# iucario/WorkoutDetector

Hardware: AMD Instinct MI355X
Metric: clips/sec (8x3x224x224 TSM-R50) (higher is better)
Workload: dtype f32

## Files before the change

### workoutdetector_amd/csrc/tsm_conv_rules.h

```cpp
#pragma once
#include <stdint.h>
#include <string.h>

#if defined(__HIPCC__)
#define TSM_HOST_DEVICE __host__ __device__
#else
#define TSM_HOST_DEVICE
#endif

namespace tsm {

struct ConvParams {
  const float *x;
  const float *w;
  const float *bias;
  const float *res;
  float *y;
  int N, Hi, Wi, C, logC4;
  int Ho, Wo, Cout;
  int stride, pad;
  int Kp;
  int M;
  int relu;
  int T;
  int fold;
  int ntm, ntn;
  int tile;
  int prec;
  const float *x2;
  int C2, Hi2, Wi2, stride2;
  int K1;
  int kseg_len;
  int ksplit;
  int tail_from;
  float *ypart;
  int reverse;
  int pos_major;
};

enum ConvPrec { kPrecF32 = 0, kPrecBf16x3 = 1, kPrecBf16 = 2 };
constexpr int kPrecBlockShift = 4;
constexpr int kPrecPosMajor = 8;

enum ConvTile {
  kTileAuto = 0, kTile128x128 = 1, kTile128x64 = 2, kTile64x64 = 3, kTile32x32 = 4,
  kTile128x128w8 = 5,
  kTile256x256 = 6,
  kTileWs = 7,
  kTile256x256p = 8,
  kTile64x128 = 9,
  kNumTiles = 10
};

struct Fused23Params {
  const float *x;
  const float *w2;
  const float *bias2;
  const float *w3f;
  const float *bias3;
  const float *res;
// ... 292 lines not shown
    case kTile64x128:
      return p.prec == kPrecF32 && p.pad == 0 && p.kseg_len == 0 && p.Cout % 128 == 0 &&
             !(p.T > 0 && (p.res || p.x2 || p.stride != 1));
    case kTileWs: {
      int tr, tc;
      return conv3x3_ws_valid(p, &tr, &tc) || conv3x3_ws128s2_valid(p, &tr, &tc) || conv3x3_ws128_valid(p, &tr, &tc, nullptr) ||
             conv1x1_ws_valid(p) || conv1x1_wsn_valid(p, n_cu);
    }
    default: return false;
  }
}

enum ConvFamily { kFamInvalid = 0, kFamIgemm, kFamIgemmSeg, kFamBf16_256, kFamBf16_256p, kFamWs3x3, kFamWs128, kFamWs128s2, kFamWs1x1, kFamWsn };

struct ConvRoute {
  int family = kFamInvalid, ks = 0;
  int bm = 0, bn = 0, wgm = 0, wgn = 0;
  bool shift = false, res = false, dual = false, block_shift = false;
  bool pos_major = false;
  int ntm = 0, ntn = 0;
  long tiles = 0;
  unsigned grid = 0;
  int tr = 0, tc = 0, swz = 0;
};

inline bool conv_args_refused(const ConvParams &p, int ks) {
  const int kc = p.prec == kPrecBf16 ? 64 : kBK;
  if (p.Cout % 64 != 0 || p.Kp % kc != 0 || p.M <= 0) return true;
  if (p.logC4 < 0 || p.logC4 > 28 || (1 << p.logC4) * 4 != p.C) return true;
  if (ks != 7 && p.C % kc != 0) return true;
  if (p.T > 0 && ((ks != 1 && ks != 3) || (ks == 3 && p.kseg_len > 0) || p.N % p.T != 0 || p.fold % 4 != 0 ||
                  (p.res && 2 * (int64_t)p.fold > p.Cout) || (p.x2 && 2 * (int64_t)p.fold > p.C2)))
    return true;
  if (p.x2 && (ks != 1 || p.res || p.K1 % kc != 0 || p.C2 % kc != 0 || (int64_t)p.K1 + p.C2 != p.Kp || p.K1 != p.C))
    return true;
  if (p.x2 && (128.0 / ((double)p.Ho * p.Wo) + 4.0) * (double)p.Hi2 * p.Wi2 * p.C2 * 4.0 > 2.0e9) return true;
  if (p.T > 0 && p.res && (128.0 + 2.0 * p.Ho * p.Wo) * p.Cout * 4.0 > 2.0e9) return true;
  if (p.prec != kPrecF32 && p.prec != kPrecBf16x3 && p.prec != kPrecBf16) return true;
  if (p.kseg_len < 0 || (p.kseg_len > 0 && (p.prec != kPrecF32 || p.res || ks == 7))) return true;
  if ((p.ksplit && p.kseg_len <= 0) || p.ksplit < 0 || p.ksplit > 2) return true;
  if (p.prec != kPrecF32 && p.T > 0 && p.fold % 8 != 0) return true;
  if (ks == 7 && (p.C != 4 || (p.prec != kPrecF32 && (p.stride != 2 || p.pad != 3)))) return true;
  if ((128.0 / ((double)p.Ho * p.Wo) + 4.0) * (double)p.Hi * p.Wi * p.C * 4.0 > 2.0e9) return true;
  return (ks != 1 && ks != 3 && ks != 7) || (ks == 7 && p.res);
}

// ... 8 lines not shown
  for (int ky = 0; ky < 3; ++ky)
    for (int kx = 0; kx < 3; ++kx)
      if ((unsigned)(iy0 + ky) < (unsigned)Hi && (unsigned)(ix0 + kx) < (unsigned)Wi) mask |= 1u << (ky * 3 + kx);
  return mask;
}
TSM_HOST_DEVICE inline int next_live_kstep(int kt, unsigned mask, int steps_per_tap, int nk) {
  if (kt < 0 || kt >= nk) return nk;
  const int log_spt = __builtin_ctz((unsigned)steps_per_tap);
  const int tap = kt >> log_spt;
  const unsigned rest = tap < 9 ? (mask & 0x1ffu) >> tap : 0u;
  if (rest & 1u) return kt;
  if (rest == 0u) return nk;
  const int next = (tap + __builtin_ctz(rest)) << log_spt;
  return next < nk ? next : nk;
}
inline bool pos_major_valid(const ConvParams &p, int ks) {
  return p.prec == kPrecF32 && ks == 3 && p.pad == 1 && (p.stride == 1 || p.stride == 2) && p.kseg_len > 0 && p.T == 0 &&
         !p.res && !p.x2 && (p.tile == kTile64x64 || p.tile == kTileAuto) && (p.ksplit == 0 || p.ksplit == 2) &&
         p.N > 0 && p.N % 64 == 0 && p.Ho > 0 && p.Wo > 0 && (int64_t)p.N * p.Ho * p.Wo == p.M &&
         p.C >= kBK && (p.C & (p.C - 1)) == 0 && p.Kp == (int64_t)9 * p.C &&
         (double)p.N * p.Hi * p.Wi * p.C * 4.0 < 2.0e9 && (double)p.M * p.Cout * 4.0 < 2.0e9;
}

inline ConvRoute conv_route(const ConvParams &p, int ks, int n_cu) {
  ConvRoute r, refused;
  if (conv_args_refused(p, ks) || (p.tile != kTileAuto && !conv_tile_valid(p, p.tile, n_cu))) return refused;
  r.ks = ks; r.res = p.res != nullptr; r.dual = p.x2 != nullptr;
  r.shift = !r.res && p.T > 0 && !(ks == 1 && r.dual);
  if (p.tile == kTileAuto) conv_tile_shape(p, &r.bm, &r.bn);
  else conv_tile_dims(p.tile, &r.bm, &r.bn);
  if (p.tile == kTile256x256 || p.tile == kTile256x256p) {
    const bool persistent = p.tile == kTile256x256p;
    if (!(persistent ? conv_bf16_256p_valid(p, ks) : conv_bf16_256_valid(p, ks))) return refused;
    r.family = persistent ? kFamBf16_256p : kFamBf16_256;
    r.wgm = 2; r.wgn = 4;
    r.shift = ks == 1 && p.T > 0;
    r.ntm = (int)(((long)p.M + 255) / 256); r.ntn = p.Cout / 256;
    r.tiles = (long)r.ntm * r.ntn;
    const int slots = n_cu & ~7;
    r.grid = (unsigned)(!persistent || r.tiles < slots || slots < 8 ? r.tiles : slots);
    return r.tiles > 0x7fffffffL ? refused : r;
  }
  if (p.tile == kTileWs) {
    if (ks == 3) {
      r.family = conv3x3_ws128s2_valid(p, &r.tr, &r.tc) ? kFamWs128s2 : conv3x3_ws128_valid(p, &r.tr, &r.tc, &r.swz) ? kFamWs128 :
                 conv3x3_ws_valid(p, &r.tr, &r.tc) ? kFamWs3x3 : kFamInvalid;
// ... 7 lines not shown
      r.tiles = ((long)p.M + px - 1) / px;
    }
    r.grid = persistent_grid(r.tiles, n_cu);
    if (r.family == kFamWsn && p.x2 && p.Kp == 384) {
      const int pairs = n_cu >> 4 << 3;
      r.grid = 2u * (unsigned)(r.tiles < pairs ? (r.tiles + 7) / 8 * 8 : pairs);
    }
    return r;
  }
  if (p.tile == kTile64x128 && ks != 1) return refused;
  if (p.kseg_len > 0 && r.bm != 32) r.bm = r.bn = 64;
  if (r.bm == 32 && p.prec != kPrecF32) return refused;
  r.wgm = r.bm == 32 ? 1 : r.bm == 128 && r.bn == 128 && p.tile == kTile128x128w8 ? 4 : 2;
  r.wgn = r.bm == 32 ? 1 : 2;
  r.ntm = (int)(((long)p.M + r.bm - 1) / r.bm); r.ntn = p.Cout / r.bn;
  r.tiles = (long)r.ntm * r.ntn;
  long grid = r.tiles;
  if (p.kseg_len > 0) {
    if (r.res || ks == 7 || (r.shift && ks == 3)) return refused;
    if (p.ksplit == 2 && (p.tail_from <= 0 || p.tail_from >= r.tiles || p.tail_from % r.ntn != 0)) return refused;
    r.family = kFamIgemmSeg;
    r.pos_major = p.pos_major != 0 && r.bm == 64 && pos_major_valid(p, ks);
    grid = p.ksplit == 2 ? p.tail_from + (r.tiles - p.tail_from) * conv_num_segments(p) : r.tiles * (p.ksplit ? conv_num_segments(p) : 1);
  } else {
    r.family = kFamIgemm;
  }
  r.block_shift = p.T > 0 && (r.dual || r.res);
  r.grid = (unsigned)grid;
  return grid > 0x7fffffffL ? refused : r;
}

inline bool conv23_ws_valid(int n, int h, int w, int *tr_out = nullptr, int *tc_out = nullptr) {
  int tr, tc;
  return n > 0 && h > 0 && w > 0 && (double)h * w * 512.0 < 2.0e9 && (double)n * h * w < 2.0e9 &&
         ws_tile_geometry(h, w, tr_out ? tr_out : &tr, tc_out ? tc_out : &tc);
}
inline bool bneck_ws_valid(int cin, int n, int h, int w, int T, int fold) {
  return (cin == 256 || cin == 64) && n > 0 && h > 0 && w >= 1 && w <= 64 && (double)h * w * 512.0 * 3.0 < 2.0e9 &&
         (T == 0 || (T > 0 && n % T == 0 && fold == cin / 8));
}
inline bool front_s2_valid(int n, int h, int w, int T, int fold) {
  return n > 0 && h >= 2 && (h & 1) == 0 && w >= 2 && w <= 64 && (double)h * w * 512.0 * 3.0 < 2.0e9 &&
         (T == 0 || (T > 0 && n % T == 0 && fold == 32));
}
inline int conv31_rows(const Conv31Params &p) {
  if (p.K3 == 128 && p.C == 512 && p.N1 == 128) return 256;
// ... 13 lines not shown
```

### workoutdetector_amd/csrc/tsm_device.h

```cpp
#pragma once
#include "tsm_kernels.h"

#include <cstdio>
#include <cstdlib>
#include <cstring>
#include <map>
#include <mutex>
#include <utility>

namespace tsm {

typedef float f32x16 __attribute__((ext_vector_type(16)));
typedef float f32x4 __attribute__((ext_vector_type(4)));
typedef float f32x2 __attribute__((ext_vector_type(2)));
typedef unsigned u32x4 __attribute__((ext_vector_type(4)));

constexpr int kLds = 36;

constexpr unsigned kInvalid = 0x80000000u;

__device__ __forceinline__ long xcd_chunked(long v, long n) {
  const long q8 = n >> 3, r8 = n & 7, x = v & 7;
  return (x < r8 ? x * (q8 + 1) : r8 * (q8 + 1) + (x - r8) * q8) + (v >> 3);
}
// ... 84 lines not shown
}
#define TSM_STAMP_DECL(on, n) \
  [[maybe_unused]] unsigned long long stamp_acc[(on) ? (n) : 1] = {}, stamp_last = (on) ? __builtin_amdgcn_s_memtime() : 0
#define TSM_STAMP(on, i)                                          \
  do {                                                            \
    if (on) {                                                     \
      const unsigned long long _t = __builtin_amdgcn_s_memtime(); \
      stamp_acc[(on) ? (i) : 0] += _t - stamp_last;               \
      stamp_last = _t;                                            \
    }                                                             \
  } while (0)

#define TSM_KLAUNCH(kern, ...)                          \
  do {                                                  \
    ::tsm::note_launch(#kern, __PRETTY_FUNCTION__);     \
    hipLaunchKernelGGL(kern, __VA_ARGS__);              \
  } while (0)
#define TSM_KLAUNCH_WALK(rev, kern, ...)                             \
  do {                                                               \
    ::tsm::note_launch(#kern, __PRETTY_FUNCTION__, (rev) ? 1 : 0);   \
    hipLaunchKernelGGL(kern, __VA_ARGS__);                           \
  } while (0)

inline unsigned grid_for(int64_t total, int cap) {
  const int64_t blocks = (total + 255) / 256;
  return (unsigned)(blocks < cap ? (blocks > 0 ? blocks : 1) : cap);
}

struct DeviceInfo {
  int n_cu = 256;
  hipError_t status = hipSuccess;
};
const DeviceInfo &device_info();
hipError_t lds_opt_in(const void *kernel, size_t bytes);
struct OptIn {
  hipError_t first = hipSuccess;
  void operator()(const void *fn, size_t bytes) {
    const hipError_t st = lds_opt_in(fn, bytes);
    if (st != hipSuccess && first == hipSuccess) first = st;
  }
};
hipError_t opt_in_bf16_256();
hipError_t opt_in_ws();
hipError_t opt_in_bneck();
hipError_t opt_in_conv31();
hipError_t opt_in_front();
// ... 7 lines not shown
```

### workoutdetector_amd/csrc/tsm_engine.hip

```cpp
#include <hip/hip_runtime.h>

#include <sys/stat.h>

#include <algorithm>
#include <cerrno>
#include <cmath>
#include <cstdio>
#include <cstdlib>
#include <cstring>
#include <map>
#include <string>
#include <vector>

#include "../../include/tsm_hip.h"
#include "tsm_host_util.h"
#include "tsm_kernels.h"

#ifndef TSM_BUILD_ID
#define TSM_BUILD_ID __DATE__ "/" __TIME__
#endif

namespace {

using namespace tsm_host;
// ... 152 lines not shown
  float *buf[5] = {nullptr, nullptr, nullptr, nullptr, nullptr};
  float *d_pooled = nullptr, *d_logits = nullptr;
  float *d_partial = nullptr;
  size_t partial_elems = 0;
  size_t buf_elems = 0;
  int h1 = 0, w1 = 0, hp = 0, wp = 0;
  hipEvent_t ev0 = nullptr, ev1 = nullptr;
  bool have_time = false;
  std::vector<void *> allocs;
  bool poison = false;
  std::vector<GuardBuf> guards;
  std::map<int, std::vector<int>> tile_cache;
  bool autotune = true;
  bool stem_pool = true;
  bool stem_direct = true;
  bool stem_planar = true;
  std::string tune_path, tune_sig;
  int force_tile = 0, force_code = -1;
  int fuse23 = -1;
  int fuse_block = -1;
  int fuse31 = -1;
  int fuse_front = -1;
  bool pos_major = true;
  bool tile_64x128 = true;
  int walk = -1;
  int n_cu = 256;
  int timing_left = 0;
  bool timing_only3x3 = false;
  std::vector<std::vector<hipEvent_t>> timing;
  std::vector<hipEvent_t> event_pool;
  std::vector<hipEvent_t> *cur_timing = nullptr;
};

namespace {

int fail(tsm_engine *e, int code, const std::string &msg) {
  if (e) e->err = msg; else g_create_error = msg;
  return code;
}

#define TSM_HIP(e, call)                                                                        \
  do {                                                                                          \
    hipError_t _st = (call);                                                                    \
    if (_st != hipSuccess)                                                                      \
      return fail((e), TSM_ERR_HIP, std::string(#call) + ": " + hipGetErrorString(_st));        \
  } while (0)
// ... 320 lines not shown
  fclose(f);
  return ok;
}

void tune_cache_store(tsm_engine *e, int key, const std::vector<int> &codes) {
  if (e->tune_path.empty()) return;
  std::string line = e->tune_sig + "|" + std::to_string(key) + "|";
  for (size_t i = 0; i < codes.size(); ++i) line += (i ? "," : "") + std::to_string(codes[i]);
  line += "\n";
  if (line.size() >= 4096) return;
  FILE *f = fopen(e->tune_path.c_str(), "a");
  if (!f) return;
  fwrite(line.data(), 1, line.size(), f);
  fclose(f);
}

bool tail_split_from(const tsm::ConvParams &p, int n_cu, size_t partial_elems, int *tail_from) {
  if (p.kseg_len <= 0) return false;
  const long from = tsm_host::tail_split_point(p.M, p.Cout, tsm::conv_num_segments(p), n_cu, partial_elems);
  *tail_from = (int)from;
  return from > 0;
}

hipError_t launch_conv_code(tsm::ConvParams p, int ks, int code, float *partial, size_t partial_elems, int n_cu, hipStream_t s) {
  p.tile = code & kCodeTileMask;
  const bool pos_major = (code & kCodePosMajor) && !(code & kCodeSplitK) && (code & kCodeTileMask) == tsm::kTile64x64 &&
                         tsm::pos_major_valid(p, ks);
  p.pos_major = pos_major ? 1 : 0;
  if ((code & kCodeSplitK) && p.kseg_len > 0 &&
      (size_t)tsm::conv_num_segments(p) * (size_t)p.M * (size_t)p.Cout <= partial_elems) {
    float *y = p.y;
    p.ksplit = 1;
    p.y = partial;
    hipError_t st = tsm::launch_conv(p, ks, s);
    if (st == hipSuccess)
      st = tsm::launch_splitk_reduce(partial, tsm::conv_num_segments(p), p.M, p.Cout, p.bias, nullptr, y, p.relu, s);
    return st;
  }
  if ((code & kCodeTailK) && (code & kCodeTileMask) == tsm::kTile64x64 && p.kseg_len > 0) {
    int tail_from = 0;
    if (tail_split_from(p, n_cu, partial_elems, &tail_from)) {
      float *y = p.y;
      const int mt0 = tail_from / (p.Cout / 64) * 64;
      p.ksplit = 2;
      p.tail_from = tail_from;
      p.ypart = partial;
      hipError_t st = tsm::launch_conv(p, ks, s);
      if (st == hipSuccess && pos_major)
        st = tsm::launch_splitk_reduce_pos(partial, tsm::conv_num_segments(p), mt0, p.M - mt0, p.N, p.Ho * p.Wo, p.Cout, p.bias, y,
                                           p.relu, s);
      else if (st == hipSuccess)
// ... 199 lines not shown
  }
  hipError_t launch_code(tsm::ConvParams p, int ks, int code);
  hipError_t launch_pair(const tsm::ConvParams &a, int ks_a, int code_a, const tsm::ConvParams &b, int ks_b, int code_b) {
    const hipError_t st = launch_code(a, ks_a, code_a);
    return st != hipSuccess ? st : launch_code(b, ks_b, code_b);
  }
  template <class A, class B>
  int fused_wins(A &&many, B &&one, bool *wins) {
    float many_ms = 0.f, one_ms = 0.f;
    int rc = time_best_of(e, s, many, &many_ms);
    if (!rc) rc = time_best_of(e, s, one, &one_ms);
    *wins = one_ms < many_ms;
    return rc;
  }
  int conv(int idx, tsm::ConvParams p, int ks, bool is3x3);
  int run_basic(size_t k, int nn, float *x, float *y, int hh, int ww);
  int run_block(size_t k, const BlockPlan &plan, int nn, float *x, float *y, int hh, int ww);
  int run_nonlocal(size_t k, int nn, float *x, float *z, int hh, int ww);
  int run_mse(size_t k, int nn, int hh, int ww);
  int tune_block(size_t k, int nn, float *x, float *y, int hh, int ww);
};

hipError_t Forward::launch_code(tsm::ConvParams p, int ks, int code) {
  return launch_conv_code(p, ks, code, e->d_partial, e->partial_elems, e->n_cu, s);
}

int Forward::conv(int idx, tsm::ConvParams p, int ks, bool is3x3) {
  p.reverse = next_dir();
  if (!tuning) {
    int code = tiles ? (*tiles)[idx] : 0;
    if (e->force_tile) code = e->force_tile;
    if (e->force_code >= 0) code = e->force_code;
    TSM_LAUNCH_K(e, s, is3x3, launch_code(p, ks, checked_code(p, code, e->n_cu)));
    return TSM_OK;
  }
  std::vector<int> cands;
  if (p.kseg_len > 0) {
    const size_t need = (size_t)tsm::conv_num_segments(p) * p.M * p.Cout;
    const long tiles64 = (long)((p.M + 63) / 64) * (p.Cout / 64);
    for (int t : {(int)tsm::kTile64x64, (int)tsm::kTile32x32}) {
      cands.push_back(t);
      if (need <= e->partial_elems && tiles64 < 4L * e->n_cu) cands.push_back(t | kCodeSplitK);
    }
    int tail_from = 0;
    const bool tail = tail_split_from(p, e->n_cu, e->partial_elems, &tail_from);
    if (tail) cands.push_back((int)tsm::kTile64x64 | kCodeTailK);
    tsm::ConvParams q = p;
// ... 905 lines not shown
    if (rows >= (int64_t)1 << 31)
      return fail(nullptr, TSM_ERR_CAPACITY, "max_clips * num_segments * (H/2) * (W/2) must stay below 2^31");
  }
  if (const char *why = shift_div_refusal(cfg->shift_div, tsm::kPrecF32)) return fail(nullptr, TSM_ERR_UNSUPPORTED, why);
  if (prec_of_dtype(cfg->dtype) < 0)
    return fail(nullptr, TSM_ERR_UNSUPPORTED, "dtype must be TSM_DTYPE_F32, TSM_DTYPE_BF16X3 or TSM_DTYPE_BF16");
  if (const char *why = shift_div_refusal(cfg->shift_div, prec_of_dtype(cfg->dtype))) return fail(nullptr, TSM_ERR_UNSUPPORTED, why);
  int ndev = 0;
  hipError_t st = hipGetDeviceCount(&ndev);
  if (st != hipSuccess || ndev <= 0)
    return fail(nullptr, TSM_ERR_HIP, std::string("no HIP device: ") + hipGetErrorString(st));
  if (cfg->device_id < 0 || cfg->device_id >= ndev) return fail(nullptr, TSM_ERR_INVALID_ARG, "bad device_id");
  tsm_engine *e = new tsm_engine();
  e->cfg = *cfg;
  e->prec = prec_of_dtype(cfg->dtype);
  const auto on = [](const char *s) { return atoi(s) != 0; };
  env_read("TSM_AUTOTUNE", &e->autotune, on);
  env_read("TSM_STEM_DIRECT", &e->stem_direct, on);
  env_read("TSM_STEM_POOL", &e->stem_pool, on);
  env_read("TSM_STEM_PLANAR", &e->stem_planar, on);
  env_read("TSM_CONV_TILE", &e->force_tile, tsm::conv_tile_from_name);
  env_read("TSM_CONV_CODE", &e->force_code, atoi);
  env_read("TSM_POS_MAJOR", &e->pos_major, on);
  env_read("TSM_TILE_64X128", &e->tile_64x128, on);
  env_read("TSM_FUSE_CONV23", &e->fuse23, on);
  env_read("TSM_FUSE_BLOCK", &e->fuse_block, on);
  env_read("TSM_FUSE_C3C1", &e->fuse31, on);
  env_read("TSM_FUSE_FRONT", &e->fuse_front, on);
  env_read("TSM_WALK", &e->walk, on);
  env_read("TSM_POISON", &e->poison, on);
  const char *tc = getenv("TSM_TUNE_CACHE");
  if (!tc) e->tune_path = default_tune_cache_path();
  else if (*tc && strcmp(tc, "0") != 0 && strcmp(tc, "off") != 0) e->tune_path = tc;
  build_topology(e);
  st = hipSetDevice(cfg->device_id);
  if (st == hipSuccess) st = hipStreamCreateWithFlags(&e->stream, hipStreamNonBlocking);
  if (st == hipSuccess) st = hipDeviceGetAttribute(&e->n_cu, hipDeviceAttributeMultiprocessorCount, cfg->device_id);
  if (st == hipSuccess) st = hipEventCreate(&e->ev0);
  if (st == hipSuccess) st = hipEventCreate(&e->ev1);
  if (st != hipSuccess) {
    g_create_error = std::string("engine init: ") + hipGetErrorString(st);
    delete e;
    return TSM_ERR_HIP;
  }
  if (!e->tune_path.empty()) {
    hipDeviceProp_t prop;
// ... 494 lines not shown
    xin = d_x4;
  } else if (x3 && (rc = staged(a->x, "d_xs", (size_t)pl.x_elems, in_px * a->cin, &xin))) {
    return rc;
  }
  if (x3) {
    if ((rc = scratch.alloc(&d_ys, "d_ys", out_elems, out_frame, act_bytes))) return rc;
    yout = d_ys;
    if (rin && (rc = staged(rin, "d_rs", out_elems, out_frame, &rin))) return rc;
    if (pl.dual && (rc = staged(x2in, "d_x2s", (size_t)pl.x2_elems, (size_t)a->hi2 * a->wi2 * a->cin2, &x2in))) return rc;
  }
  tsm::ConvParams p = make_params(c, xin, rin, yout, n, hi, wi, a->relu != 0, pl.T, 1, prec);
  p.fold = pl.fold;
  p.reverse = a->reverse != 0;
  if (pl.dual) set_second_source(&p, c2.kp, x2in, a->cin2, a->hi2, a->wi2, a->stride2);
  int dev = 0, n_cu = 256;
  TSM_HIP(nullptr, hipGetDevice(&dev));
  TSM_HIP(nullptr, hipDeviceGetAttribute(&n_cu, hipDeviceAttributeMultiprocessorCount, dev));
  const int code = checked_code(p, a->code > 0 ? a->code & ~kCodeOpSegmented : a->code, n_cu);
  size_t part_elems = 0;
  if ((code & (kCodeSplitK | kCodeTailK)) && p.kseg_len > 0) {
    part_elems = (size_t)tsm::conv_num_segments(p) * p.M * p.Cout;
    if ((rc = scratch.alloc(&d_part, "d_part", part_elems, out_frame))) return rc;
  }
  const char *sd_env = getenv("TSM_STEM_DIRECT");
  hipError_t st;
  if (pl.stem && x3 && cout == 64 && !(sd_env && atoi(sd_env) == 0))
    st = tsm::launch_stem_direct(xin, c.d_w, c.d_b, yout, n, hi, wi, c.kp, a->relu != 0, prec, s);
  else
    st = launch_conv_code(p, a->k, code, d_part, part_elems, n_cu, s);
  if (st == hipSuccess && x3) st = tsm::launch_to_f32(d_ys, a->y, (int64_t)out_elems / 8, prec, s);
  const hipError_t st2 = hipStreamSynchronize(s);
  if (st != hipSuccess) return op_status("launch_conv", st);
  if (st2 != hipSuccess) return fail(nullptr, TSM_ERR_HIP, std::string("conv sync: ") + hipGetErrorString(st2));
  for (int i = 0; i < scratch.n; ++i) {
    std::string msg;
    TSM_HIP(nullptr, guard_verify(scratch.g[i], &msg));
    if (!msg.empty()) return fail(nullptr, TSM_ERR_GUARD, "tsm_conv_op: " + msg);
  }
  return TSM_OK;
}

int tsm_conv_bn_act(const float *x, const float *w, const float *gamma, const float *beta, const float *mean,
                    const float *var, const float *residual, float *y, int32_t n, int32_t hi, int32_t wi,
                    int32_t cin, int32_t cout, int32_t k, int32_t stride, int32_t relu, int32_t shift_segments,
                    int32_t fold_div, int32_t dtype, void *stream) {
  tsm_conv_args a{};
  a.struct_size = sizeof(tsm_conv_args);
  a.x = x; a.w = w; a.gamma = gamma; a.beta = beta; a.mean = mean; a.var = var; a.residual = residual; a.y = y;
  a.n = n; a.hi = hi; a.wi = wi; a.cin = cin; a.cout = cout; a.k = k; a.stride = stride; a.relu = relu;
  a.shift_segments = shift_segments; a.fold_div = fold_div; a.dtype = dtype;
  a.code = tsm::conv_tile_from_name(getenv("TSM_CONV_TILE"));
  return tsm_conv_op(&a, stream);
// ... 229 lines not shown
```

### workoutdetector_amd/csrc/tsm_igemm.hip

```cpp
#include "tsm_device.h"

namespace tsm {

template <int BM, int BN, int WGM, int WGN, int KS, bool SHIFT, bool RES, int PREC, bool DUAL = false, bool SEG = false>
__global__ void __launch_bounds__(64 * WGM * WGN, (SEG && BM == 64) ? ((PREC & kPrecBlockShift) ? 4 : 5) : (BM == 64 && BN == 128) ? 4 : 1)
conv_igemm(const ConvParams p) {
  constexpr bool BSHIFT = (PREC & kPrecBlockShift) != 0;
  constexpr bool POSM = (PREC & kPrecPosMajor) != 0;
  constexpr int PMODE = PREC & ~(kPrecBlockShift | kPrecPosMajor);
  static_assert(!POSM || (SEG && KS == 3 && BM == 64 && BN == 64 && !SHIFT && !RES && !DUAL && !BSHIFT && PMODE == kPrecF32),
                "position-major rows: the segmented fp32 3x3 on 64x64 tiles only (pos_major_valid)");
  static_assert(!BSHIFT || (!SHIFT && !RES), "block placement: a shifted identity (DUAL = false) or a shifted second source");
  constexpr bool RESID = RES || (BSHIFT && !DUAL);
  static_assert(!SEG || (PMODE == kPrecF32 && !RES && WGM * WGN <= 4 && BM == BN && BM <= 64),
                "segmented K accumulation: fp32, 64x64 / 32x32 tiles, no residual (ConvParams::kseg_len)");
  static_assert(WGM * WGN == 4 || WGM * WGN == 1 || WGM * WGN == 8,
                "4 waves per workgroup, 1 (32x32 small-M tiles) or 8 (128x128 with 4 waves per SIMD at 2 workgroups/CU)");
  constexpr int NT = 64 * WGM * WGN;
  constexpr int LRP = NT / 8;
  static_assert(!DUAL || (KS == 1 && !SHIFT && !RES), "K-concatenated second source: plain 1x1 convs only");
  constexpr bool X3 = PMODE == kPrecBf16x3;
  constexpr bool BF = PMODE == kPrecBf16;
  constexpr int EB = BF ? 2 : 4;
  constexpr int KC = 128 / EB;
  static_assert(!SHIFT || KS == 1 || (KS == 3 && !SEG), "the temporal shift is fused into 1x1 and unsegmented 3x3 convs only");
  constexpr int WTM = BM / WGM, WTN = BN / WGN;
  constexpr int TM = WTM / 32, TN = WTN / 32;
  constexpr int APASS = BM / LRP, BPASS = BN / LRP;
  constexpr bool RK = PMODE == kPrecF32 && ((BM == 64 && BN == 64) || (BM == 32 && BN == 32));
  constexpr bool RK2 = PMODE == kPrecF32 && BM == 64 && BN == 128;
  static_assert(!RK2 || (WGM == 2 && WGN == 2 && KS == 1 && !SEG && !BSHIFT && !POSM),
                "64x128 tiles: unsegmented fp32 1x1 convs on 2x2 waves, no block placement (conv_tile_valid)");
  constexpr int NBUF = (RK || RK2) ? 1 : 2;
  constexpr int CLD = RK2 ? 68 : BN + 4;
  static_assert(TM >= 1 && TN >= 1, "wave tile must hold at least one 32x32 MFMA tile");
  constexpr int SMEM_FLOATS = NBUF * (BM + BN) * kLds > BM * CLD ? NBUF * (BM + BN) * kLds : BM * CLD;

  __shared__ __attribute__((aligned(16))) float smem[SMEM_FLOATS];

  const int tid = threadIdx.x;
  const int lane = tid & 63;
  const int wave = tid >> 6;
  const int wm = wave / WGN, wn = wave % WGN;
  const int half = lane >> 5, l31 = lane & 31;

  const int bid = blockIdx.x;
  const bool tail_mode = SEG && p.ksplit == 2;
  const bool in_tail = tail_mode && bid >= p.tail_from;
  const int nwg = tail_mode ? p.tail_from : (int)gridDim.x;
  const int q = nwg >> 3, r = nwg & 7, xcd = bid & 7;
  int tile = (xcd < r ? xcd * (q + 1) : r * (q + 1) + (xcd - r) * q) + (bid >> 3);
  if (p.reverse) tile = nwg - 1 - tile;
  int seg = 0;
  if (SEG && p.ksplit == 1) {
    seg = tile / (p.ntm * p.ntn);
    tile -= seg * (p.ntm * p.ntn);
  }
  if (in_tail) {
    const int u = bid - p.tail_from, n_tail = p.ntm * p.ntn - p.tail_from;
    seg = u / n_tail;
    tile = p.tail_from + (u - seg * n_tail);
  }
  const bool split_wg = SEG && (p.ksplit == 1 || in_tail);
  const int tm = tile / p.ntn, tn = tile - tm * p.ntn;
  const int m0 = tm * BM, n0 = tn * BN;

  const int HoWo = p.Ho * p.Wo;
  const int n_first = POSM ? 0 : m0 / HoWo;
  const int frame0 = SHIFT ? (n_first > 0 ? n_first - 1 : 0) : n_first;
  constexpr bool PAIRS = KS == 7 && PMODE != kPrecF32;
  const int wpairs = (p.Wi + 1) >> 1;
  const size_t frame_elems = PAIRS ? (size_t)p.Hi * wpairs * 8 : (size_t)p.Hi * p.Wi * p.C;
  const size_t a_bytes = ((size_t)p.N - frame0) * frame_elems * EB;
  const __amdgpu_buffer_rsrc_t rsrcA = buffer_window(reinterpret_cast<const char *>(p.x) + (size_t)frame0 * frame_elems * EB, a_bytes);
  const __amdgpu_buffer_rsrc_t rsrcB = buffer_fixed(reinterpret_cast<const char *>(p.w) + (size_t)n0 * p.Kp * EB, BN * p.Kp * EB);

  const size_t frame_elems2 = DUAL ? (size_t)p.Hi2 * p.Wi2 * p.C2 : 0;
  const int frame02 = (BSHIFT && DUAL && n_first > 0) ? n_first - 1 : n_first;
  const size_t a2_bytes = DUAL ? ((size_t)p.N - frame02) * frame_elems2 * EB : 0;
  const __amdgpu_buffer_rsrc_t rsrcA2 = buffer_window(reinterpret_cast<const char *>(DUAL ? p.x2 : p.x) + (size_t)frame02 * frame_elems2 * EB, a2_bytes);

  const int lrow = tid >> 3;
// ... 681 lines not shown
    else TSM_KLAUNCH_WALK_X(p.reverse, ARM(kPrecF32), grid, block, 0, s, p);                            \
    return hipGetLastError();                                                                           \
  } while (0)
#define TSM_ARM_DUAL_SHIFT(PREC) (conv_igemm<BM, BN, WGM, WGN, 1, false, false, PREC | kPrecBlockShift, true>)
#define TSM_ARM_DUAL(PREC) (conv_igemm<BM, BN, WGM, WGN, 1, false, false, PREC, true>)
#define TSM_ARM_RES_SHIFT(PREC) (conv_igemm<BM, BN, WGM, WGN, KS, false, false, PREC | kPrecBlockShift>)
#define TSM_ARM_PLAIN(PREC) (conv_igemm<BM, BN, WGM, WGN, KS, SHIFT, RES, PREC>)

template <int BM, int BN, int WGM, int WGN, int KS, bool SHIFT>
static hipError_t launch_conv_seg(const ConvParams &p, const ConvRoute &r, hipStream_t s) {
  if constexpr (!((BM == 64 && BN == 64) || (BM == 32 && BN == 32))) {
    return hipErrorInvalidValue;
  } else {
    const dim3 grid(r.grid), block(64 * WGM * WGN);
    if constexpr (KS == 1 && !SHIFT) {
      if (r.dual) {
        if (r.block_shift) TSM_KLAUNCH_WALK(p.reverse, (conv_igemm<BM, BN, WGM, WGN, 1, false, false, kPrecF32 | kPrecBlockShift, true, true>), grid, block, 0, s, p);
        else TSM_KLAUNCH_WALK(p.reverse, (conv_igemm<BM, BN, WGM, WGN, 1, false, false, kPrecF32, true, true>), grid, block, 0, s, p);
        return hipGetLastError();
      }
    }
    if constexpr (BM == 64 && WGM == 2 && KS == 3 && !SHIFT) {
      if (r.pos_major) {
        TSM_KLAUNCH_WALK(p.reverse, (conv_igemm<64, 64, 2, 2, 3, false, false, kPrecF32 | kPrecPosMajor, false, true>), grid, block, 0, s, p);
        return hipGetLastError();
      }
    }
    TSM_KLAUNCH_WALK(p.reverse, (conv_igemm<BM, BN, WGM, WGN, KS, SHIFT, false, kPrecF32, false, true>), grid, block, 0, s, p);
    return hipGetLastError();
  }
}

template <int BM, int BN, int WGM, int WGN, int KS, bool SHIFT, bool RES>
static hipError_t launch_conv_t(const ConvParams &p, const ConvRoute &r, hipStream_t s) {
  if (r.family == kFamIgemmSeg) {
    if constexpr (!RES && KS != 7 && !(SHIFT && KS == 3)) return launch_conv_seg<BM, BN, WGM, WGN, KS, SHIFT>(p, r, s);
    else return hipErrorInvalidValue;
  }
  const dim3 grid(r.grid), block(64 * WGM * WGN);
  if constexpr (KS == 1 && !SHIFT && !RES) {
    if (r.dual && r.block_shift) TSM_LAUNCH_IGEMM_AND_RETURN(TSM_ARM_DUAL_SHIFT);
    if (r.dual) TSM_LAUNCH_IGEMM_AND_RETURN(TSM_ARM_DUAL);
  }
  if constexpr (RES && !SHIFT && KS != 7) {
    if (r.block_shift) TSM_LAUNCH_IGEMM_AND_RETURN(TSM_ARM_RES_SHIFT);
  }
  TSM_LAUNCH_IGEMM_AND_RETURN(TSM_ARM_PLAIN);
// ... 6 lines not shown
  else if (r.res) TSM_KLAUNCH_WALK(p.reverse, (conv_igemm<64, 128, 2, 2, 1, false, true, kPrecF32>), grid, block, 0, s, p);
  else if (r.shift) TSM_KLAUNCH_WALK(p.reverse, (conv_igemm<64, 128, 2, 2, 1, true, false, kPrecF32>), grid, block, 0, s, p);
  else TSM_KLAUNCH_WALK(p.reverse, (conv_igemm<64, 128, 2, 2, 1, false, false, kPrecF32>), grid, block, 0, s, p);
  return hipGetLastError();
}

template <int KS, bool SHIFT, bool RES>
static hipError_t launch_conv_ks(const ConvParams &p, const ConvRoute &r, hipStream_t s) {
  if (r.bm == 32) return launch_conv_t<32, 32, 1, 1, KS, SHIFT, RES>(p, r, s);
  if (r.bm == 128 && r.bn == 128 && r.wgm == 4) return launch_conv_t<128, 128, 4, 2, KS, SHIFT, RES>(p, r, s);
  if (r.bm == 128 && r.bn == 128) return launch_conv_t<128, 128, 2, 2, KS, SHIFT, RES>(p, r, s);
  if (r.bm == 128) return launch_conv_t<128, 64, 2, 2, KS, SHIFT, RES>(p, r, s);
  return launch_conv_t<64, 64, 2, 2, KS, SHIFT, RES>(p, r, s);
}

hipError_t launch_conv(const ConvParams &p_in, int ks, hipStream_t s) {
  const bool device = p_in.tile == kTile256x256 || p_in.tile == kTile256x256p || p_in.tile == kTileWs;
  const DeviceInfo *di = device ? &device_info() : nullptr;
  const ConvRoute r = conv_route(p_in, ks, di ? di->n_cu : 0);
  if (r.family == kFamInvalid) return hipErrorInvalidValue;
  if (di && di->status != hipSuccess) return di->status;
  ConvParams p = p_in;
  p.ntm = r.ntm; p.ntn = r.ntn;
  if (r.family == kFamBf16_256 || r.family == kFamBf16_256p) return launch_conv_bf16_256(p, r, s);
  if (r.family >= kFamWs3x3) return launch_conv_ws(p, r, s);
  if (p.ksplit == 2 && !p.ypart) return hipErrorInvalidValue;
  if (r.bm == 64 && r.bn == 128) return launch_conv_64x128(p, r, s);
  if (ks == 1) return r.res ? launch_conv_ks<1, false, true>(p, r, s) : r.shift ? launch_conv_ks<1, true, false>(p, r, s) : launch_conv_ks<1, false, false>(p, r, s);
  if (ks == 3) return r.res ? launch_conv_ks<3, false, true>(p, r, s) : r.shift ? launch_conv_ks<3, true, false>(p, r, s) : launch_conv_ks<3, false, false>(p, r, s);
  return launch_conv_ks<7, false, false>(p, r, s);
}

__global__ void __launch_bounds__(256) splitk_reduce_kernel(const float *__restrict__ partial, int n_seg, int64_t n4,
                                                            int64_t seg_stride4, int cout4,
                                                            const float *__restrict__ bias, const float *__restrict__ res,
                                                            float *__restrict__ y, int relu) {
  const int64_t stride = (int64_t)gridDim.x * blockDim.x;
  const float floor_ = relu ? 0.f : -INFINITY;
  const f32x4 *p4 = reinterpret_cast<const f32x4 *>(partial);
  for (int64_t i = (int64_t)blockIdx.x * blockDim.x + threadIdx.x; i < n4; i += stride) {
    f32x4 t = p4[i];
    for (int sgm = 1; sgm < n_seg; ++sgm) t += p4[i + sgm * seg_stride4];
    f32x4 v = t + reinterpret_cast<const f32x4 *>(bias)[i % cout4];
    if (res) v += reinterpret_cast<const f32x4 *>(res)[i];
    v[0] = fmaxf(v[0], floor_);
    v[1] = fmaxf(v[1], floor_);
// ... 51 lines not shown
```

### workoutdetector_amd/csrc/tsm_kernels.h

```cpp
#pragma once
#include <hip/hip_runtime.h>
#include <stdint.h>

#include "tsm_conv_rules.h"

namespace tsm_host {
struct TdnPoolSource;
}

namespace tsm {

hipError_t launch_conv(const ConvParams &p, int ks, hipStream_t s);
hipError_t launch_conv23_fused(const Fused23Params &p, int cmid, int cout3, int prec, hipStream_t s);
hipError_t launch_bneck_ws(const BneckParams &p, hipStream_t s);
hipError_t launch_front_s2(const FrontParams &p, hipStream_t s);
hipError_t launch_conv31_fused(const Conv31Params &p, hipStream_t s);

hipError_t launch_stem_direct(const float *x, const float *w, const float *bias, float *y, int n, int hi, int wi, int kp,
                              int relu, int prec, hipStream_t s);
hipError_t launch_stem_pool(const float *x, const float *w, const float *bias, float *y, int n, int hi, int wi, int kp,
                            int relu, int prec, hipStream_t s, int planar = 0);
hipError_t launch_splitk_reduce(const float *partial, int n_seg, int64_t m, int cout, const float *bias,
                                const float *res, float *y, int relu, hipStream_t s);
hipError_t launch_splitk_reduce_pos(const float *partial, int n_seg, int64_t m_first, int64_t m, int n_frames, int howo, int cout,
// ... 109 lines not shown
hipError_t launch_layer_norm(const float *x, const float *ln_w, const float *ln_b, float *y, int64_t rows, int c, hipStream_t s);
hipError_t launch_layer_norm_s2d(const float *x, const float *ln_w, const float *ln_b, float *y, int n, int h, int w, int c, hipStream_t s);
hipError_t launch_stem_pack4(const float *x, float *y, int n, int h, int w, hipStream_t s);
hipError_t launch_gelu(float *x, int64_t n4, hipStream_t s);

hipError_t launch_tdn_front(const float *x, float *in4, float *patches, int n_frames, int h, int w, hipStream_t s);
hipError_t launch_tdn_front_pool(const tsm_host::TdnPoolSource &src, float *in4, float *patches, int n_segments, int h, int w, hipStream_t s);
hipError_t launch_tdn_fuse(float *x, const float *d, int n, int h, int w, int hd, int wd, int c, float alpha, float beta, hipStream_t s);
hipError_t launch_tdn_fuse_ring(const float *ring_a, const float *ring_d, const int32_t *table, int n_slots, float *x, int n, int h, int w,
                                int hd, int wd, int c, float alpha, float beta, hipStream_t s);
hipError_t launch_mse_squeeze(const float *x, const float *wq, const float *bq, float *b, int64_t m, int c, hipStream_t s);
hipError_t launch_mse_diff(const float *b, const float *dw, float *df, float *db, float *pf, float *pb, int n_frames, int T, int h, int w,
                           int c, hipStream_t s);
hipError_t launch_mse_s2(const float *pf, const float *pb, const float *k2, const float *b2, float *sf, float *sb, int n_frames, int hp, int wp,
                         int c, hipStream_t s);
hipError_t launch_mse_mix(const float *df, const float *db, const float *s2f, const float *s2b, const float *k4, const float *b4, float *mf,
                          float *mb, int n_frames, int h, int w, int c, hipStream_t s);
hipError_t launch_mse_excite_shift(const float *x, const float *mf, const float *mb, const float *w3, const float *b3, const float *wt, float *o,
                                   int n_clips, int T, int hw, int c, hipStream_t s);

hipError_t launch_scores_to_states(const float *logits, int n, int c, int softmax, float threshold, int *states, float *top,
                                   hipStream_t s);

void note_launch(const char *kernel, const char *where, int reverse = -1);
void trace_launches(bool on);
const char *launch_trace();

}
```

### workoutdetector_amd/csrc/tsm_ops.hip

```cpp
#include "tsm_device.h"
#include "tsm_host_util.h"

#include <string>

namespace tsm {

template <int FMT>
struct Fmt {
  static constexpr int ch = FMT == kPrecF32 ? 4 : 8;
  static constexpr int gf = FMT == kPrecBf16x3 ? 8 : 4;
};

template <int FMT>
__device__ __forceinline__ void load_group(const float *p, float v[8]) {
  if (FMT == kPrecF32) {
    const f32x4 a = *reinterpret_cast<const f32x4 *>(p);
#pragma unroll
    for (int e = 0; e < 4; ++e) {
      v[e] = a[e];
      v[e + 4] = 0.f;
    }
  } else if (FMT == kPrecBf16x3) {
    const u32x4 h = *reinterpret_cast<const u32x4 *>(p), l = *reinterpret_cast<const u32x4 *>(p + 4);
#pragma unroll
// ... 1280 lines not shown
  if (t < c) {
    correct[t] += n_correct[t];
    total[t] += n_total[t];
  }
}

hipError_t launch_top1_tally(const float *logits, const int *labels, int n, int c, int *pred, int *correct, int *total,
                             hipStream_t s) {
  if (!logits || !labels || !correct || !total || n <= 0 || c <= 0) return hipErrorInvalidValue;
  if (c > kTallyMaxClass) return hipErrorNotSupported;
  TSM_KLAUNCH(top1_tally_kernel, dim3(1), dim3(kTallyMaxClass), 0, s, logits, labels, n, c, pred, correct, total);
  return hipGetLastError();
}


namespace {
struct LaunchTrace {
  bool on = false;
  std::string text;
};
thread_local LaunchTrace g_trace;
}

void note_launch(const char *kernel, const char *where, int reverse) {
  if (!g_trace.on) return;
  std::string k(kernel);
  if (!k.empty() && k.front() == '(' && k.back() == ')') k = k.substr(1, k.size() - 2);
  const char *with = where ? strstr(where, " [") : nullptr;
  g_trace.text += k;
  if (with) g_trace.text += with;
  if (reverse > 0) g_trace.text += " [reverse]";
  g_trace.text += '\n';
}
void trace_launches(bool on) {
  g_trace.on = on;
  if (on) g_trace.text.clear();
}
const char *launch_trace() { return g_trace.text.c_str(); }

hipError_t lds_opt_in(const void *kernel, size_t bytes) {
  return hipFuncSetAttribute(kernel, hipFuncAttributeMaxDynamicSharedMemorySize, (int)bytes);
}

const DeviceInfo &device_info() {
  static std::mutex mu;
  static std::map<int, DeviceInfo> seen;
  int dev = 0;
  (void)hipGetDevice(&dev);
  std::lock_guard<std::mutex> lock(mu);
  auto it = seen.find(dev);
  if (it != seen.end()) return it->second;
  DeviceInfo di;
  hipDeviceProp_t prop;
// ... 8 lines not shown
```

Baseline: 1915.

## Balance position-major 3x3 conv tiles across XCDs by live-tap cost

For position-major segmented 3x3 convolutions, computes per-tile cost from the popcount of live kernel taps at each output position and partitions whole tiles into eight contiguous runs with roughly equal cost, one per XCD. The kernel maps each block to its XCD's run and returns early for padded slots, so the grid is enlarged to eight times the longest run. This targets imbalance where border positions skip taps and some XCDs finish early, at the cost of idle launched blocks and a longer host-side routing pass. It is enabled by default and can be turned off with an environment variable.

```diff
diff --git a/workoutdetector_amd/csrc/tsm_conv_rules.h b/workoutdetector_amd/csrc/tsm_conv_rules.h
--- a/workoutdetector_amd/csrc/tsm_conv_rules.h
+++ b/workoutdetector_amd/csrc/tsm_conv_rules.h
@@ -36,6 +36,9 @@
   float *ypart;
   int reverse;
   int pos_major;
+  int pos_balance;
+  int pos_whole;
+  int pos_run[9];
 };
 
 enum ConvPrec { kPrecF32 = 0, kPrecBf16x3 = 1, kPrecBf16 = 2 };
@@ -374,6 +377,7 @@
   long tiles = 0;
   unsigned grid = 0;
   int tr = 0, tc = 0, swz = 0;
+  int pos_whole = 0, pos_run[9] = {0, 0, 0, 0, 0, 0, 0, 0, 0};
 };
 
 inline bool conv_args_refused(const ConvParams &p, int ks) {
@@ -428,6 +432,36 @@
          (double)p.N * p.Hi * p.Wi * p.C * 4.0 < 2.0e9 && (double)p.M * p.Cout * 4.0 < 2.0e9;
 }
 
+constexpr int kXcds = 8;
+inline int pos_balanced_runs(const ConvParams &p, int ntn, long nwg, int run[kXcds + 1]) {
+  const int groups = (int)(nwg / ntn), per_pos = p.N / 64;
+  int cached_pos = -1, cached_cost = 0;
+  auto cost = [&](int g) {
+    const int pos = g / per_pos;
+    if (pos != cached_pos) {
+      cached_pos = pos;
+      cached_cost = __builtin_popcount(pos_major_tap_mask(pos, p.Wo, p.Hi, p.Wi, p.stride, p.pad));
+    }
+    return cached_cost;
+  };
+  long total = 0;
+  for (int g = 0; g < groups; ++g) total += cost(g);
+  long cum = 0;
+  int g = 0, longest = 0;
+  run[0] = 0;
+  for (int k = 1; k <= kXcds; ++k) {
+    int b = groups;
+    if (k < kXcds) {
+      while (g < groups && cum * kXcds < k * total) cum += cost(g++);
+      b = g;
+      if (g > 0 && k * total - (cum - cost(g - 1)) * kXcds < cum * kXcds - k * total) b = g - 1;
+    }
+    run[k] = b * ntn;
+    if (run[k] - run[k - 1] > longest) longest = run[k] - run[k - 1];
+  }
+  return kXcds * longest;
+}
+
 inline ConvRoute conv_route(const ConvParams &p, int ks, int n_cu) {
   ConvRoute r, refused;
   if (conv_args_refused(p, ks) || (p.tile != kTileAuto && !conv_tile_valid(p, p.tile, n_cu))) return refused;
@@ -481,6 +515,11 @@
     r.family = kFamIgemmSeg;
     r.pos_major = p.pos_major != 0 && r.bm == 64 && pos_major_valid(p, ks);
     grid = p.ksplit == 2 ? p.tail_from + (r.tiles - p.tail_from) * conv_num_segments(p) : r.tiles * (p.ksplit ? conv_num_segments(p) : 1);
+    if (r.pos_major && p.pos_balance) {
+      const long whole = p.ksplit == 2 ? p.tail_from : r.tiles;
+      r.pos_whole = pos_balanced_runs(p, r.ntn, whole, r.pos_run);
+      grid += r.pos_whole - whole;
+    }
   } else {
     r.family = kFamIgemm;
   }
diff --git a/workoutdetector_amd/csrc/tsm_device.h b/workoutdetector_amd/csrc/tsm_device.h
--- a/workoutdetector_amd/csrc/tsm_device.h
+++ b/workoutdetector_amd/csrc/tsm_device.h
@@ -130,6 +130,12 @@
     hipLaunchKernelGGL(kern, __VA_ARGS__);                           \
   } while (0)
 
+#define TSM_KLAUNCH_WALK_MARK(rev, mark, kern, ...)                          \
+  do {                                                                       \
+    ::tsm::note_launch(#kern, __PRETTY_FUNCTION__, (rev) ? 1 : 0, (mark));   \
+    hipLaunchKernelGGL(kern, __VA_ARGS__);                                   \
+  } while (0)
+
 inline unsigned grid_for(int64_t total, int cap) {
   const int64_t blocks = (total + 255) / 256;
   return (unsigned)(blocks < cap ? (blocks > 0 ? blocks : 1) : cap);
diff --git a/workoutdetector_amd/csrc/tsm_engine.hip b/workoutdetector_amd/csrc/tsm_engine.hip
--- a/workoutdetector_amd/csrc/tsm_engine.hip
+++ b/workoutdetector_amd/csrc/tsm_engine.hip
@@ -198,6 +198,7 @@
   int fuse31 = -1;
   int fuse_front = -1;
   bool pos_major = true;
+  bool pos_balance = true;
   bool tile_64x128 = true;
   int walk = -1;
   int n_cu = 256;
@@ -564,11 +565,13 @@
   return from > 0;
 }
 
-hipError_t launch_conv_code(tsm::ConvParams p, int ks, int code, float *partial, size_t partial_elems, int n_cu, hipStream_t s) {
+hipError_t launch_conv_code(tsm::ConvParams p, int ks, int code, float *partial, size_t partial_elems, int n_cu, hipStream_t s,
+                            bool pos_balance = true) {
   p.tile = code & kCodeTileMask;
   const bool pos_major = (code & kCodePosMajor) && !(code & kCodeSplitK) && (code & kCodeTileMask) == tsm::kTile64x64 &&
                          tsm::pos_major_valid(p, ks);
   p.pos_major = pos_major ? 1 : 0;
+  p.pos_balance = pos_major && pos_balance ? 1 : 0;
   if ((code & kCodeSplitK) && p.kseg_len > 0 &&
       (size_t)tsm::conv_num_segments(p) * (size_t)p.M * (size_t)p.Cout <= partial_elems) {
     float *y = p.y;
@@ -814,7 +817,7 @@
 };
 
 hipError_t Forward::launch_code(tsm::ConvParams p, int ks, int code) {
-  return launch_conv_code(p, ks, code, e->d_partial, e->partial_elems, e->n_cu, s);
+  return launch_conv_code(p, ks, code, e->d_partial, e->partial_elems, e->n_cu, s, e->pos_balance);
 }
 
 int Forward::conv(int idx, tsm::ConvParams p, int ks, bool is3x3) {
@@ -1766,6 +1769,7 @@
   env_read("TSM_CONV_TILE", &e->force_tile, tsm::conv_tile_from_name);
   env_read("TSM_CONV_CODE", &e->force_code, atoi);
   env_read("TSM_POS_MAJOR", &e->pos_major, on);
+  env_read("TSM_POS_BALANCE", &e->pos_balance, on);
   env_read("TSM_TILE_64X128", &e->tile_64x128, on);
   env_read("TSM_FUSE_CONV23", &e->fuse23, on);
   env_read("TSM_FUSE_BLOCK", &e->fuse_block, on);
@@ -2306,12 +2310,12 @@
     part_elems = (size_t)tsm::conv_num_segments(p) * p.M * p.Cout;
     if ((rc = scratch.alloc(&d_part, "d_part", part_elems, out_frame))) return rc;
   }
-  const char *sd_env = getenv("TSM_STEM_DIRECT");
+  const char *sd_env = getenv("TSM_STEM_DIRECT"), *pb_env = getenv("TSM_POS_BALANCE");
   hipError_t st;
   if (pl.stem && x3 && cout == 64 && !(sd_env && atoi(sd_env) == 0))
     st = tsm::launch_stem_direct(xin, c.d_w, c.d_b, yout, n, hi, wi, c.kp, a->relu != 0, prec, s);
   else
-    st = launch_conv_code(p, a->k, code, d_part, part_elems, n_cu, s);
+    st = launch_conv_code(p, a->k, code, d_part, part_elems, n_cu, s, !(pb_env && atoi(pb_env) == 0));
   if (st == hipSuccess && x3) st = tsm::launch_to_f32(d_ys, a->y, (int64_t)out_elems / 8, prec, s);
   const hipError_t st2 = hipStreamSynchronize(s);
   if (st != hipSuccess) return op_status("launch_conv", st);
diff --git a/workoutdetector_amd/csrc/tsm_igemm.hip b/workoutdetector_amd/csrc/tsm_igemm.hip
--- a/workoutdetector_amd/csrc/tsm_igemm.hip
+++ b/workoutdetector_amd/csrc/tsm_igemm.hip
@@ -46,18 +46,30 @@
 
   const int bid = blockIdx.x;
   const bool tail_mode = SEG && p.ksplit == 2;
-  const bool in_tail = tail_mode && bid >= p.tail_from;
-  const int nwg = tail_mode ? p.tail_from : (int)gridDim.x;
+  bool balanced = false;
+  if constexpr (POSM) balanced = p.pos_whole > 0;
+  const int whole = balanced ? p.pos_whole : p.tail_from;
+  const bool in_tail = tail_mode && bid >= whole;
+  const int nwg = tail_mode ? p.tail_from : balanced ? p.ntm * p.ntn : (int)gridDim.x;
   const int q = nwg >> 3, r = nwg & 7, xcd = bid & 7;
   int tile = (xcd < r ? xcd * (q + 1) : r * (q + 1) + (xcd - r) * q) + (bid >> 3);
-  if (p.reverse) tile = nwg - 1 - tile;
+  bool mirror = p.reverse != 0;
+  if constexpr (POSM) {
+    if (balanced && !in_tail) {
+      const int run = p.reverse ? 7 - xcd : xcd, first = p.pos_run[run], len = p.pos_run[run + 1] - first, idx = bid >> 3;
+      if (idx >= len) return;
+      tile = p.reverse ? first + len - 1 - idx : first + idx;
+      mirror = false;
+    }
+  }
+  if (mirror) tile = nwg - 1 - tile;
   int seg = 0;
   if (SEG && p.ksplit == 1) {
     seg = tile / (p.ntm * p.ntn);
     tile -= seg * (p.ntm * p.ntn);
   }
   if (in_tail) {
-    const int u = bid - p.tail_from, n_tail = p.ntm * p.ntn - p.tail_from;
+    const int u = bid - whole, n_tail = p.ntm * p.ntn - p.tail_from;
     seg = u / n_tail;
     tile = p.tail_from + (u - seg * n_tail);
   }
@@ -785,7 +797,10 @@
     }
     if constexpr (BM == 64 && WGM == 2 && KS == 3 && !SHIFT) {
       if (r.pos_major) {
-        TSM_KLAUNCH_WALK(p.reverse, (conv_igemm<64, 64, 2, 2, 3, false, false, kPrecF32 | kPrecPosMajor, false, true>), grid, block, 0, s, p);
+        char mark[48];
+        snprintf(mark, sizeof mark, " [balanced %d/%ld]", p.pos_whole, p.ksplit == 2 ? (long)p.tail_from : r.tiles);
+        TSM_KLAUNCH_WALK_MARK(p.reverse, p.pos_whole > 0 ? mark : nullptr,
+                              (conv_igemm<64, 64, 2, 2, 3, false, false, kPrecF32 | kPrecPosMajor, false, true>), grid, block, 0, s, p);
         return hipGetLastError();
       }
     }
@@ -838,6 +853,8 @@
   if (di && di->status != hipSuccess) return di->status;
   ConvParams p = p_in;
   p.ntm = r.ntm; p.ntn = r.ntn;
+  p.pos_whole = r.pos_whole;
+  for (int k = 0; k <= kXcds; ++k) p.pos_run[k] = r.pos_run[k];
   if (r.family == kFamBf16_256 || r.family == kFamBf16_256p) return launch_conv_bf16_256(p, r, s);
   if (r.family >= kFamWs3x3) return launch_conv_ws(p, r, s);
   if (p.ksplit == 2 && !p.ypart) return hipErrorInvalidValue;
diff --git a/workoutdetector_amd/csrc/tsm_kernels.h b/workoutdetector_amd/csrc/tsm_kernels.h
--- a/workoutdetector_amd/csrc/tsm_kernels.h
+++ b/workoutdetector_amd/csrc/tsm_kernels.h
@@ -155,7 +155,7 @@
 hipError_t launch_scores_to_states(const float *logits, int n, int c, int softmax, float threshold, int *states, float *top,
                                    hipStream_t s);
 
-void note_launch(const char *kernel, const char *where, int reverse = -1);
+void note_launch(const char *kernel, const char *where, int reverse = -1, const char *mark = nullptr);
 void trace_launches(bool on);
 const char *launch_trace();
 
diff --git a/workoutdetector_amd/csrc/tsm_ops.hip b/workoutdetector_amd/csrc/tsm_ops.hip
--- a/workoutdetector_amd/csrc/tsm_ops.hip
+++ b/workoutdetector_amd/csrc/tsm_ops.hip
@@ -1326,13 +1326,14 @@
 thread_local LaunchTrace g_trace;
 }
 
-void note_launch(const char *kernel, const char *where, int reverse) {
+void note_launch(const char *kernel, const char *where, int reverse, const char *mark) {
   if (!g_trace.on) return;
   std::string k(kernel);
   if (!k.empty() && k.front() == '(' && k.back() == ')') k = k.substr(1, k.size() - 2);
   const char *with = where ? strstr(where, " [") : nullptr;
   g_trace.text += k;
   if (with) g_trace.text += with;
+  if (mark) g_trace.text += mark;
   if (reverse > 0) g_trace.text += " [reverse]";
   g_trace.text += '\n';
 }
```

New measurement: 1940, median of 6. +1.3%, better.
